# luoao-kddi/SCP

Measured on AMD Instinct MI355X. Metric: KITTI frames/sec encode (SCP-EHEM, level 16) + bpp match vs ref, higher is better.
Workload: dtype f32 (dense layers and attention as bf16x3 split on bf16 MFMA, feature kNN as f16x3 split on f16 MFMA, fp32 accumulate; position kNN / CDF in fp32); 1 GPU; SCP-EHEM KITTI-like synthetic 120k-pt frames, --spher --mullevel lidar_level=16 (BASELINE.json configs[2]), seeded random weights; nodes_per_frame=577403, windows_per_frame=100, frames_per_gpu=46, frames_in_flight=4, frames_per_launch_sequence=1, transform=host-numpy on a prefetch thread (strict identity: the reference's integers), parallelism=frame-sharded x1, rank_cores=256, rank_cores_pinned=False

## Files before the change

include/scp.h:

```cpp
#ifndef SCP_H
#define SCP_H
#include <stddef.h>
#include <stdint.h>

#ifdef __cplusplus
extern "C" {
#endif

#define SCP_API __attribute__((visibility("default")))

#define SCP_OK 0
#define SCP_EINVAL (-1)
#define SCP_ENOMEM (-2)
#define SCP_ESMALL (-3)
#define SCP_EHIP (-4)
#define SCP_ESTATE (-5)

#define SCP_MAX_DEPTH 21
#define SCP_MAX_SEGMENTS 62

#define SCP_ABI_VERSION 220
SCP_API int scp_version(void);
SCP_API int scp_last_hip_error(void);
SCP_API int scp_device_count(void);
// ... 338 lines not shown
    double mn, den;
} scp_expand_seg;
SCP_API int scp_decode_expand_batch(const int64_t *sym, const int64_t *cum, const int32_t *pos, const uint8_t *anc, const uint8_t *octant,
                                    int64_t n, const scp_expand_seg *seg, int32_t S, int32_t cs, const int64_t *wbase, int32_t K, int64_t M,
                                    int64_t T, void *table_dev, int32_t *cpos, uint8_t *canc, uint8_t *coct, uint8_t *cctx, float *cposn,
                                    uint8_t *occ8, void *stream);

SCP_API int scp_swin_ln_linear(const float *x, int64_t ldx, const float *valid, const void *Whi, const void *Wlo, const float *bias,
                               const float *wbeta, float eps, float *out, int64_t ldo, int32_t M, int32_t N, void *stream);
SCP_API int scp_swin_post_attn(const void *Ohi, const void *Olo, int64_t ldo_in, const float *x, int64_t ldx, const void *W, const float *bp,
                               const float *b1, const float *b2, float eps, float *out, int64_t ldc, int32_t M, const int32_t *tile_list,
                               int32_t n_tiles, void *stream);
SCP_API int64_t scp_swin_post_attn_weight_bytes(void);
SCP_API double scp_gelu_prescale(void);

SCP_API int scp_swin_merge(const float *x, int64_t ldx, int64_t n_src, const int64_t *ia, const int64_t *ib, const void *W, const float *wbeta,
                           float eps, float *out, int64_t ldo, int32_t M, void *stream);

SCP_API int scp_geo_edge_mlps(const float *pos1, int64_t ld1, const float *pos2, int64_t ld2, const float *pos3, int64_t ld3, const void *W,
                              const float *bias, float *out, int64_t ldo, int32_t M, void *stream);
SCP_API int scp_mlp3_rows(const float *x, int64_t ldx, int64_t n_src, const int64_t *in_map, const void *W, const float *bias, float *out, int64_t ldo,
                          const int64_t *out_map, int32_t M, int32_t N, void *stream);

SCP_API int scp_swin_kv_planes(const float *k, const float *v, int64_t ldkv, int64_t rows, void *khi, void *klo, void *vthi, void *vtlo, void *stream);
SCP_API int scp_swin_ln_qkv(const float *x, int64_t ldx, const float *valid, const void *Whi, const void *Wlo, const float *bias, const float *wbeta,
                            float eps, float *q, int64_t ldq, void *planes, int64_t Tp, int32_t M, int32_t N, void *stream);
SCP_API int scp_swin_attention_packed_planes(const float *q, const void *khi, const void *klo, const void *vthi, const void *vtlo,
                                             const float *bias_table, const int32_t *wtab, int32_t total_windows, int32_t shift, int32_t ldq,
                                             float *out, void *ohi, void *olo, int64_t ldo, const float *valid, void *stream);

#ifdef __cplusplus
}
#endif
#endif
```

scp_amd/csrc/attn.hip:

```cpp
#include <stdlib.h>
#include "scp_internal.h"

typedef float f32x16 __attribute__((ext_vector_type(16)));

#define WIN 512
#define HD 64
#define NH 4
#define QT 128
#define KT 64
#define LDK 68

typedef __bf16 bf16x4s __attribute__((ext_vector_type(4)));
__device__ __forceinline__ void store_split4(__bf16 *hi, __bf16 *lo, float a, float b, float c, float d) {
    float f[4] = {a, b, c, d};
#pragma unroll
    for (int u = 0; u < 4; ++u) asm volatile("" : "+v"(f[u]));
    bf16x4s vh, vl;
#pragma unroll
    for (int u = 0; u < 4; ++u) {
        const __bf16 hh = (__bf16)f[u];
        vh[u] = hh;
        vl[u] = (__bf16)(f[u] - (float)hh);
    }
    *(bf16x4s *)hi = vh;
// ... 218 lines not shown
#pragma unroll
        for (int j = 0; j < 8; ++j) {
            const float x = f[j] * (0.125f * LOG2E);
            const __bf16 hh = (__bf16)x;
            qh[c][j] = hh;
            ql[c][j] = (__bf16)(x - (float)hh);
        }
    }
}

__device__ __forceinline__ void attn_store_o(const f32x16 &o0, const f32x16 &o1, float inv, int h, float *dst ,
                                             __bf16 *ohi, __bf16 *olo ) {
#pragma unroll
    for (int g = 0; g < 4; ++g) {
        const int d = 8 * g + 4 * h;
        if (ohi) {
            store_split4(ohi + d, olo + d, o0[4 * g] * inv, o0[4 * g + 1] * inv, o0[4 * g + 2] * inv, o0[4 * g + 3] * inv);
            store_split4(ohi + 32 + d, olo + 32 + d, o1[4 * g] * inv, o1[4 * g + 1] * inv, o1[4 * g + 2] * inv, o1[4 * g + 3] * inv);
        } else {
            *(float4 *)(dst + d) = make_float4(o0[4 * g] * inv, o0[4 * g + 1] * inv, o0[4 * g + 2] * inv, o0[4 * g + 3] * inv);
            *(float4 *)(dst + 32 + d) = make_float4(o1[4 * g] * inv, o1[4 * g + 1] * inv, o1[4 * g + 2] * inv, o1[4 * g + 3] * inv);
        }
    }
}

template <bool FASTFIRST>
__global__ __launch_bounds__(256, 2) void swin_attn_bf16x3_kernel(const float *__restrict__ q, const float *__restrict__ k,
                                                                 const float *__restrict__ v, const float *__restrict__ table,
                                                                 int Lp, int shift, int ldq, int ldkv, float *__restrict__ out,
                                                                 const int *__restrict__ wtab, __bf16 *__restrict__ ohi,
                                                                 __bf16 *__restrict__ olo, int64_t ldo) {
    __shared__ __attribute__((aligned(16))) __bf16 Kh[KT * LDB], Kl[KT * LDB];
    __shared__ __attribute__((aligned(16))) __bf16 Vh[HD * LDB], Vl[HD * LDB];
    __shared__ float tab[2 * WIN - 1];

    const int tid = threadIdx.x, w = tid >> 6, lane = tid & 63, col = lane & 31, h = lane >> 5;
    int bid = blockIdx.x;
    bid = (bid & 7) * (int)(gridDim.x >> 3) + (bid >> 3);
    const int qtile = bid & 3; bid >>= 2;
    const int head = bid & 3; bid >>= 2;
    size_t seq_row;
    int wnd, nW;
    if (wtab) { seq_row = (size_t)wtab[2 * bid]; Lp = wtab[2 * bid + 1]; nW = Lp / WIN; wnd = (int)(((size_t)bid * WIN - seq_row) / WIN); }
    else { nW = Lp / WIN; wnd = bid % nW; seq_row = (size_t)(bid / nW) * Lp; }
    const size_t base = seq_row * (NH * HD) + head * HD;
    const size_t qbase = seq_row * ldq + head * HD, kbase = seq_row * ldkv + head * HD;
// ... 149 lines not shown
        for (int t = 0; t < WIN / PKT; ++t) {
            if (PNS > 2 && t + 1 < WIN / PKT) SCP_BARRIER_DMA(4); else SCP_BARRIER_DMA(0);
            if (t + PNS - 1 < WIN / PKT) issue(t + PNS - 1, (t + PNS - 1) % PNS);
            const char *S = stg + (t % PNS) * PST;
            const float madd = (masked && ((t * PKT) >> 8) != qreg) ? -100.f * LOG2E : 0.f;
            auto kfrag = [&](int c, bf16x8 &ah, bf16x8 &al) {
                const int ko = col * 128 + (((2 * c + h) ^ (col & 7)) << 4);
                ah = *(const bf16x8 *)(S + ko); al = *(const bf16x8 *)(S + 4096 + ko);
            };
            auto vfrag = [&](int c, bf16x8 &v0h, bf16x8 &v0l, bf16x8 &v1h, bf16x8 &v1l) {
                const int R0 = col >> 1, R1 = R0 + 16, sl = (col & 1) * 4 + 2 * c + h;
                const int v0 = R0 * 128 + ((sl ^ (R0 & 7)) << 4), v1 = R1 * 128 + ((sl ^ (R1 & 7)) << 4);
                v0h = *(const bf16x8 *)(S + 8192 + v0); v0l = *(const bf16x8 *)(S + 12288 + v0);
                v1h = *(const bf16x8 *)(S + 8192 + v1); v1l = *(const bf16x8 *)(S + 12288 + v1);
            };
            attn_tile<FAST>(kfrag, vfrag, qh, ql, tab, qi - (t * PKT + 4 * h) + (WIN - 1), madd, h, o0, o1, m_run, l_run);
        }
    };
    if (FASTFIRST) {
        sweep(AttnFast{});
        if (__syncthreads_or(!attn_fast_ok(l_run, o0, o1, h))) sweep(AttnStd{});
    } else sweep(AttnStd{});
    const float inv = 1.0f / l_run;
    attn_store_o(o0, o1, inv, h, out ? out + base + (size_t)qtok * (NH * HD) : nullptr,
                 ohi ? ohi + (seq_row + (size_t)qtok) * (size_t)ldo + head * HD : nullptr, ohi ? olo + (seq_row + (size_t)qtok) * (size_t)ldo + head * HD : nullptr);
}

__global__ __launch_bounds__(256) void kv_planes_kernel(const float *__restrict__ k, const float *__restrict__ v, int64_t ldkv, int64_t rows,
                                                       __bf16 *__restrict__ khi, __bf16 *__restrict__ klo, __bf16 *__restrict__ vthi,
                                                       __bf16 *__restrict__ vtlo) {
    const int64_t g = (int64_t)blockIdx.x * 256 + threadIdx.x;
    if (g >= rows * 32) return;
    const int64_t row = g >> 5;
    const int head = (int)(g >> 3) & 3, ch = (int)g & 7;
    const float *ks = k + row * ldkv + head * HD + 8 * ch, *vs = v + row * ldkv + head * HD + 8 * ch;
    const float4 a = *(const float4 *)ks, b = *(const float4 *)(ks + 4), c = *(const float4 *)vs, d = *(const float4 *)(vs + 4);
    const float kf[8] = {a.x, a.y, a.z, a.w, b.x, b.y, b.z, b.w}, vf[8] = {c.x, c.y, c.z, c.w, d.x, d.y, d.z, d.w};
    bf16x8 kh, kl;
#pragma unroll
    for (int u = 0; u < 8; ++u) { const __bf16 hh = (__bf16)kf[u]; kh[u] = hh; kl[u] = (__bf16)(kf[u] - (float)hh); }
    const int64_t ko = row * (NH * HD) + head * HD + ((ch ^ (int)(row & 7)) << 3);
    *(bf16x8 *)(khi + ko) = kh;
    *(bf16x8 *)(klo + ko) = kl;
    const int kk = (int)(row & 31), p = (kk & ~12) | ((kk & 4) << 1) | ((kk & 8) >> 1);
    const int64_t vb = ((row >> 5) * NH + head) * (int64_t)2048;
#pragma unroll
// ... 6 lines not shown
    }
}

extern "C" SCP_API int scp_swin_kv_planes(const float *k, const float *v, int64_t ldkv, int64_t rows, void *khi, void *klo, void *vthi, void *vtlo,
                                          void *stream) {
    if (!k || !v || !khi || !klo || !vthi || !vtlo || rows <= 0 || (rows & 31) || ldkv < NH * HD || (ldkv & 3) ||
        (((uintptr_t)k | (uintptr_t)v | (uintptr_t)khi | (uintptr_t)klo | (uintptr_t)vthi | (uintptr_t)vtlo) & 15))
        return SCP_EINVAL;
    hipLaunchKernelGGL(kv_planes_kernel, dim3((unsigned)cdiv64(rows * 32, 256)), dim3(256), 0, (hipStream_t)stream, k, v, ldkv, rows, (__bf16 *)khi,
                       (__bf16 *)klo, (__bf16 *)vthi, (__bf16 *)vtlo);
    LAUNCH_CHECK();
    return SCP_OK;
}

static std::atomic<int> g_attn_variant{1};
extern "C" SCP_API int scp_set_attention_variant(int32_t v) { g_attn_variant.store(v ? 1 : 0, std::memory_order_relaxed); return SCP_OK; }
extern "C" SCP_API int scp_get_attention_variant(void) { return g_attn_variant.load(std::memory_order_relaxed); }

extern "C" SCP_API int scp_swin_attention_packed_planes(const float *q, const void *khi, const void *klo, const void *vthi, const void *vtlo,
                                                        const float *bias_table, const int32_t *wtab, int32_t total_windows, int32_t shift, int32_t ldq,
                                                        float *out, void *ohi, void *olo, int64_t ldo, const float *valid, void *stream) {
    if (!q || !khi || !klo || !vthi || !vtlo || !bias_table || !wtab || (!out && !ohi) || total_windows <= 0 || (shift != 0 && shift != WIN / 2) ||
        ldq < NH * HD || (ldq & 3) || (((uintptr_t)q | (uintptr_t)out | (uintptr_t)khi | (uintptr_t)klo | (uintptr_t)vthi | (uintptr_t)vtlo) & 15) ||
        (ohi && (!olo || ldo < NH * HD || (ldo & 3) || (((uintptr_t)ohi | (uintptr_t)olo) & 7))))
        return SCP_EINVAL;
    SCP_PROF(SCP_PROF_ATTENTION, stream, (double)total_windows * WIN * 2.0 * 2.0 * WIN * NH * HD);
#define ATTN_GO(V) hipLaunchKernelGGL(swin_attn_planes_kernel<V>, dim3(total_windows * NH * (WIN / QT)), dim3(256), PNS * PST, (hipStream_t)stream, q, (const __bf16 *)khi, \
                                      (const __bf16 *)klo, (const __bf16 *)vthi, (const __bf16 *)vtlo, bias_table, shift, ldq, out, wtab, (__bf16 *)ohi, (__bf16 *)olo, ldo, valid)
    if (g_attn_variant.load(std::memory_order_relaxed) == 0) ATTN_GO(false); else ATTN_GO(true);
#undef ATTN_GO
    LAUNCH_CHECK();
    return SCP_OK;
}

static int g_attn_mode = -1;
static inline bool attn_bf16x3() {
    const int c = scp_ctx_attention_mode();
    if (c >= 0) return c == 1;
    if (g_attn_mode < 0) { const char *e = getenv("SCP_ATTN"); g_attn_mode = (e && e[0] == 'f') ? 0 : 1; }
    return g_attn_mode == 1;
}
extern "C" SCP_API int scp_set_attention_mode(int32_t bf16x3) { g_attn_mode = bf16x3 ? 1 : 0; return SCP_OK; }

static int attn_packed(const float *q, const float *k, const float *v, const float *bias_table, const int32_t *wtab, int32_t total_windows,
                       int32_t shift, int32_t ldq, int32_t ldkv, float *out, __bf16 *ohi, __bf16 *olo, int64_t ldo, void *stream) {
    if (!q || !k || !v || !bias_table || (!out && !ohi) || !wtab || total_windows <= 0 || (shift != 0 && shift != WIN / 2) || ldq < NH * HD ||
        ldkv < NH * HD || (ldq & 3) || (ldkv & 3) || (((uintptr_t)q | (uintptr_t)k | (uintptr_t)v | (uintptr_t)out) & 15) ||
// ... 49 lines not shown
```

scp_amd/csrc/rowchain.hip:

```cpp
#include <stdlib.h>
#include "scp_internal.h"
#include "rc_common.h"

#define RC_SLOT 32768
#define RC_RING (4 * RC_SLOT)
#define RC_OFF_BOUNCE RC_RING
#define RC_OFF_BIAS (RC_RING + 4 * RC_BOUNCE)
#define RC_LDS (RC_OFF_BIAS + 16384)

__device__ __forceinline__ void rc_issue_rowchunk(const RcLane &L, const __bf16 *Whi, const __bf16 *Wlo, int g, char *slot) {
#pragma unroll
    for (int j = 0; j < 4; ++j) {
        const int p = L.w + 4 * j;
        const int64_t off = ((int64_t)g * 16 + p) * 512 + L.lane * 8;
        rc_dma16(Whi + off, slot + p * 1024);
        rc_dma16(Wlo + off, slot + 16384 + p * 1024);
    }
}

__device__ __forceinline__ void rc_issue_kchunk(const RcLane &L, const __bf16 *Whi, const __bf16 *Wlo, int c, int nks, char *slot) {
#pragma unroll
    for (int j = 0; j < 4; ++j) {
        const int p = L.w + 4 * j;
        const int64_t off = ((int64_t)p * nks + c) * 512 + L.lane * 8;
// ... 548 lines not shown
            if (gap == 5) RC_MFMA_AVV(Y[blk], A[s & 1][2], Hch[t]);
            RC_SB;
            if (s < 15 && RC_PROBE_FRAG_ON) {
                if (gap == 0 && HAS_P1) RC_DS_READ(A[nb][1], (ns & 1) ? f.r1 : f.r0, 16384 + (ns >> 1) * 1024);
                if (gap == 1) RC_DS_READ(A[nb][3], (ns & 1) ? f.k1 : f.k0, RC_SLOT + 16384 + (ns >> 1) * 2048);
                if (gap == 2 && HAS_P1) RC_DS_READ(A[nb][0], (ns & 1) ? f.r1 : f.r0, (ns >> 1) * 1024);
                if (gap == 3) RC_DS_READ(A[nb][2], (ns & 1) ? f.k1 : f.k0, RC_SLOT + (ns >> 1) * 2048);
            }
            if (RC_DMA_HERE(s, gap) && RC_PROBE_DMA_ON) rc_dma_piece(L, wr, RC_DMA_SLOT(s, gap) ? n1 : n0, nxt + RC_DMA_SLOT(s, gap) * RC_SLOT, RC_DMA_IDX(s, gap), RC_DMA_PLANE(s, gap));
            if (HAS_GELU) {
                const int k = s >> 1, st = (s & 1) * 6 + gap;
                unsigned wh = 0, wl = 0;
                rc_gelu_stage(st, g, a1g[2 * k], a1g[2 * k + 1], wh, wl);
                if (st == 10) Hnh[k >> 2][k & 3] = wh;
                if (st == 11) Hnl[k >> 2][k & 3] = wl;
            }
            RC_SB;
        }
    }
    if (NEXT == 0) RC_DS_READ4_WAIT(A[0][1], fn.r0, 16384, A[0][3], fn.k0, RC_SLOT + 16384, A[0][0], fn.r0, 0, A[0][2], fn.k0, RC_SLOT);
    else RC_DS_READ4_WAIT(A[0][1], fn.r0, 16384, A[0][3], fn.r0, RC_SLOT + 16384, A[0][0], fn.r0, 0, A[0][2], fn.r0, RC_SLOT);
}

__global__ __launch_bounds__(256, 1) void rc_post_attn_kernel(const RcPostArgs a) {
    extern __shared__ __attribute__((aligned(1024))) char smem[];
    const RcLane L = rc_lane();
    const int ntiles = (a.M + RC_ROWS - 1) / RC_ROWS;
    float *sbp = (float *)(smem + RC_OFF_BIAS), *sb2 = sbp + 256, *sb1 = sbp + 512;
    for (int i = threadIdx.x; i < 256; i += 256) { sbp[i] = a.bp[i]; sb2[i] = a.b2[i]; }
    for (int i = threadIdx.x; i < 1024; i += 256) sb1[i] = a.b1[i];
    __syncthreads();
    const int nlist = a.tile_list ? a.n_list : ntiles;
    auto tile_of = [&](int i) { return a.tile_list ? a.tile_list[i] : i; };
    int ti = blockIdx.x;
    if (ti >= nlist) return;
    int tile = tile_of(ti);
    char *bounce = smem + RC_OFF_BOUNCE + L.w * RC_BOUNCE;
    const int ldc_bytes = (int)(a.ldc * 4);
    const int voff = (32 * L.w + (L.lane >> 3)) * ldc_bytes + (L.lane & 7) * 16;

    const __amdgpu_buffer_rsrc_t wr = __builtin_amdgcn_make_buffer_rsrc((void *)a.W, 0, 2 * RC_W_PLANE, 0x00020000);
    auto src_p = [&](int g) { RcSlotSrc r = {RC_W_PROJ + g * 16384, 1024}; return r; };
    auto src_1 = [&](int c) { RcSlotSrc r = {RC_W_FC1 + c * 16384, 1024}; return r; };
    auto src_2 = [&](int c) { RcSlotSrc r = {RC_W_FC2 + c * 1024, 32 * 1024}; return r; };

    unsigned long long t_p0 = 0, t_ln = 0, t_mlp = 0, t_epi = 0, t_prev = 0, n_tiles = 0;
    const bool DBG = a.dbg != nullptr;
    unsigned long long t_first = 0, r_first = 0;
    if (DBG) { t_prev = t_first = __builtin_amdgcn_s_memtime(); r_first = __builtin_amdgcn_s_memrealtime(); }
    auto stamp = [&](unsigned long long &acc_t) { if (DBG) { const unsigned long long t = __builtin_amdgcn_s_memtime(); acc_t += t - t_prev; t_prev = t; } };

    {
        const RcSlotSrc s0 = src_p(0), s1 = src_p(1);
#pragma unroll
        for (int q = 0; q < 4; ++q)
#pragma unroll
            for (int plane = 0; plane < 2; ++plane) { rc_dma_piece(L, wr, s0, smem, q, plane); rc_dma_piece(L, wr, s1, smem + RC_SLOT, q, plane); }
    }
    rbf16x8 Bh[16], Bl[16];
    auto load_o = [&](int t) {
        const int r0 = t * RC_ROWS + 32 * L.w + (L.lane >> 3);
#pragma unroll
        for (int it = 0; it < 4; ++it) {
            const int r = r0 + 8 * it;
            const int64_t o = (int64_t)(r < a.M ? r : a.M - 1) * a.ldo_in + (L.lane & 7) * 8;
#pragma unroll
            for (int pp = 0; pp < 4; ++pp) { Bh[4 * pp + it] = *(const rbf16x8 *)(a.Ohi + o + 64 * pp); Bl[4 * pp + it] = *(const rbf16x8 *)(a.Olo + o + 64 * pp); }
        }
    };
    auto transpose_o = [&]() {
#pragma unroll
        for (int plane = 0; plane < 2; ++plane)
#pragma unroll
            for (int pp = 0; pp < 4; ++pp) {
#pragma unroll
                for (int it = 0; it < 4; ++it) {
                    const int rho = 8 * it + (L.lane >> 3), kap = L.lane & 7;
                    *(rbf16x8 *)(bounce + rho * 128 + ((kap ^ (rho & 7)) << 4)) = plane ? Bl[4 * pp + it] : Bh[4 * pp + it];
                }
                asm volatile("s_waitcnt lgkmcnt(0)" ::: "memory");
#pragma unroll
                for (int q = 0; q < 4; ++q) {
                    const rbf16x8 fr = *(const rbf16x8 *)(bounce + L.col * 128 + (((2 * q + L.h) ^ (L.col & 7)) << 4));
                    if (plane) Bl[4 * pp + q] = fr; else Bh[4 * pp + q] = fr;
                }
                asm volatile("s_waitcnt lgkmcnt(0)" ::: "memory");
            }
    };
    load_o(tile);
    transpose_o();
    rbf16x8 A[2][4];
    {
        SCP_BARRIER_DMA(0);
// ... 156 lines not shown
#pragma unroll
                for (int u = 0; u < 4; ++u) o[q][u] = Y[b][4 * q + u];
            rc_store_block(L, bounce, o, rs, ldc_bytes, voff, 32 * b);
        }
        transpose_o();
        stamp(t_epi);
        ++n_tiles;
    }
    if (DBG && L.lane == 0) {
        unsigned long long *o = a.dbg + ((size_t)blockIdx.x * 4 + L.w) * 8;
        o[0] = t_p0; o[1] = t_mlp; o[2] = t_ln; o[3] = t_epi; o[4] = n_tiles;
        o[5] = __builtin_amdgcn_s_memtime() - t_first; o[6] = __builtin_amdgcn_s_memrealtime() - r_first;
    }
    SCP_WAIT_DMA(0);
}

#ifndef RCW_D1
#define RCW_D1 4
#endif
#ifndef RCW_D2
#define RCW_D2 2
#endif
#define RCW_H_BYTES (32 * 4096)
__global__ __launch_bounds__(256, 1) void rc_post_attn_wide_kernel(const RcPostArgs a) {
    extern __shared__ __attribute__((aligned(1024))) char smem[];
    const RcLane L = rc_lane();
    float *sbp = (float *)(smem + RC_OFF_BIAS), *sb2 = sbp + 256, *sb1 = sbp + 512;
    for (int i = threadIdx.x; i < 256; i += 256) { sbp[i] = a.bp[i]; sb2[i] = a.b2[i]; }
    for (int i = threadIdx.x; i < 1024; i += 256) sb1[i] = a.b1[i];
    __syncthreads();
    const int n128 = a.tile_list ? a.n_list : (a.M + RC_ROWS - 1) / RC_ROWS;
    char *bounce = smem + RC_OFF_BOUNCE + L.w * RC_BOUNCE;
    char *hbuf = smem;
    const int ldc_bytes = (int)(a.ldc * 4);
    const int voff = (L.lane >> 3) * ldc_bytes + (L.lane & 7) * 16;
    const __amdgpu_buffer_rsrc_t wr = __builtin_amdgcn_make_buffer_rsrc((void *)a.W, 0, 2 * RC_W_PLANE, 0x00020000);
    const int vrc0 = L.rg * 8192 + L.frag, vrc1 = L.rg * 8192 + (L.frag ^ 32);
    const int vkc0 = L.rg * 32768 + L.frag, vkc1 = L.rg * 32768 + (L.frag ^ 32);
    auto wload = [&](int voff, int soff) { return __builtin_bit_cast(rbf16x8, __builtin_amdgcn_raw_buffer_load_b128(wr, voff, soff, 0)); };
    for (int item = blockIdx.x; item < 4 * n128; item += gridDim.x) {
        const int t128 = a.tile_list ? a.tile_list[item >> 2] : (item >> 2);
        const int m0 = t128 * RC_ROWS + 32 * (item & 3);
        if (m0 >= a.M) continue;
        rbf16x8 Bh[16], Bl[16];
        {
            const int r0 = m0 + (L.lane >> 3);
#pragma unroll
            for (int it = 0; it < 4; ++it) {
                const int r = r0 + 8 * it;
                const int64_t o = (int64_t)(r < a.M ? r : a.M - 1) * a.ldo_in + (L.lane & 7) * 8;
#pragma unroll
                for (int pp = 0; pp < 4; ++pp) { Bh[4 * pp + it] = *(const rbf16x8 *)(a.Ohi + o + 64 * pp); Bl[4 * pp + it] = *(const rbf16x8 *)(a.Olo + o + 64 * pp); }
            }
#pragma unroll
            for (int plane = 0; plane < 2; ++plane)
#pragma unroll
                for (int pp = 0; pp < 4; ++pp) {
#pragma unroll
                    for (int it = 0; it < 4; ++it) {
                        const int rho = 8 * it + (L.lane >> 3), kap = L.lane & 7;
                        *(rbf16x8 *)(bounce + rho * 128 + ((kap ^ (rho & 7)) << 4)) = plane ? Bl[4 * pp + it] : Bh[4 * pp + it];
                    }
                    asm volatile("s_waitcnt lgkmcnt(0)" ::: "memory");
#pragma unroll
                    for (int q = 0; q < 4; ++q) {
                        const rbf16x8 fr = *(const rbf16x8 *)(bounce + L.col * 128 + (((2 * q + L.h) ^ (L.col & 7)) << 4));
                        if (plane) Bl[4 * pp + q] = fr; else Bh[4 * pp + q] = fr;
                    }
// ... 629 lines not shown
        (q && (int64_t)RC_ROWS * ldq * 4 > 0x7fffffffLL) || 4 * Tp * 512 > 0x7fffffffLL)
        return SCP_EINVAL;
    static bool configured = false;
    if (!configured) {
        HIP_TRY(hipFuncSetAttribute((const void *)rc_ln_linear_kernel<0, true>, hipFuncAttributeMaxDynamicSharedMemorySize, RC_LDS));
        configured = true;
    }
    RcLnLinArgs a;
    a.x = x; a.ldx = ldx; a.valid = valid; a.Whi = (const __bf16 *)Whi; a.Wlo = (const __bf16 *)Wlo; a.bias = bias; a.wbeta = wbeta;
    a.out = q; a.ldo = q ? ldq : 256; a.M = M; a.N = N; a.eps = eps; a.probe = 0; a.dbg = nullptr;
    a.planes = (__bf16 *)planes; a.plane_bytes = Tp * 512; a.nq = N / 64 - 8;
    const int ntiles = M / RC_ROWS, ncu = rc_num_cu();
    SCP_PROF(SCP_PROF_LN_LINEAR, stream, 2.0 * M * 256.0 * N);
    if (rc_lnlin2_here(ntiles, ncu)) return scp_lnlin2_launch(a, true, ncu, (hipStream_t)stream);
    a.ngroups = rc_ll_groups(ntiles, N / 64, ncu);
    hipLaunchKernelGGL((rc_ln_linear_kernel<0, true>), dim3((unsigned)(a.ngroups > 1 ? ntiles * a.ngroups : (ntiles < ncu ? ntiles : ncu))), dim3(256), RC_LDS, (hipStream_t)stream, a);
    LAUNCH_CHECK();
    return SCP_OK;
}

extern "C" SCP_API int scp_swin_post_attn(const void *Ohi, const void *Olo, int64_t ldo_in, const float *x, int64_t ldx, const void *W, const float *bp,
                                          const float *b1, const float *b2, float eps, float *out, int64_t ldc, int32_t M, const int32_t *tile_list,
                                          int32_t n_tiles, void *stream) {
    if (!Ohi || !Olo || !x || !W || !bp || !b1 || !b2 || !out || M <= 0 || (tile_list && (n_tiles <= 0 || n_tiles > (M + RC_ROWS - 1) / RC_ROWS)) || ldo_in < 256 || (ldo_in & 7) || ldx < 256 || (ldx & 3) || ldc < 256 ||
        (ldc & 3) || (((uintptr_t)Ohi | (uintptr_t)Olo | (uintptr_t)x | (uintptr_t)out | (uintptr_t)W) & 15) ||
        (int64_t)RC_ROWS * ldc * 4 > 0x7fffffffLL)
        return SCP_EINVAL;
    static bool configured = false;
    if (!configured) {
        HIP_TRY(hipFuncSetAttribute((const void *)rc_post_attn_kernel, hipFuncAttributeMaxDynamicSharedMemorySize, RC_LDS));
        HIP_TRY(hipFuncSetAttribute((const void *)rc_post_attn_wide_kernel, hipFuncAttributeMaxDynamicSharedMemorySize, RC_LDS));
        configured = true;
    }
    RcPostArgs a;
    a.Ohi = (const __bf16 *)Ohi; a.Olo = (const __bf16 *)Olo; a.ldo_in = ldo_in; a.x = x; a.ldx = ldx; a.W = W;
    a.bp = bp; a.b1 = b1; a.b2 = b2; a.out = out; a.ldc = ldc; a.M = M; a.eps = eps;
    a.dbg = g_rc_dbg;
    { const char *e = getenv("SCP_RC_DUMP"); a.dbg_mode = e ? atoi(e) : 0; }
    a.tile_list = tile_list; a.n_list = tile_list ? n_tiles : 0;
    const int ntiles = tile_list ? n_tiles : (M + RC_ROWS - 1) / RC_ROWS;
    const int ncu = rc_num_cu();
    SCP_PROF(SCP_PROF_POST_ATTN, stream, 2.0 * (tile_list ? (double)n_tiles * RC_ROWS : (double)M) * (256.0 * 256.0 + 2.0 * 256.0 * 1024.0));
    if (rc_wide_mode() == 1 || (rc_wide_mode() < 0 && !g_rc_dbg && !a.dbg_mode && 4 * (int64_t)ntiles <= (int64_t)ncu)) {
        const int items = 4 * ntiles;
        hipLaunchKernelGGL(rc_post_attn_wide_kernel, dim3((unsigned)(items < 2 * ncu ? items : 2 * ncu)), dim3(256), RC_LDS, (hipStream_t)stream, a);
        LAUNCH_CHECK();
        return SCP_OK;
    }
    hipLaunchKernelGGL(rc_post_attn_kernel, dim3((unsigned)(ntiles < ncu ? ntiles : ncu)), dim3(256), RC_LDS, (hipStream_t)stream, a);
    LAUNCH_CHECK();
    return SCP_OK;
}

extern "C" SCP_API int64_t scp_swin_post_attn_weight_bytes(void) { return 2 * (int64_t)RC_W_PLANE; }

extern "C" SCP_API int scp_geo_edge_mlps(const float *pos1, int64_t ld1, const float *pos2, int64_t ld2, const float *pos3, int64_t ld3, const void *W,
                                         const float *bias, float *out, int64_t ldo, int32_t M, void *stream) {
    if (!pos1 || !pos2 || !pos3 || !W || !bias || !out || M <= 0 || ld1 < 64 || ld2 < 128 || ld3 < 256 || ((ld1 | ld2 | ld3) & 3) || ldo < 128 || (ldo & 3) ||
        (((uintptr_t)pos1 | (uintptr_t)pos2 | (uintptr_t)pos3 | (uintptr_t)out | (uintptr_t)W) & 15) || (int64_t)RC_ROWS * ldo * 4 > 0x7fffffffLL)
        return SCP_EINVAL;
    static bool configured = false;
    if (!configured) {
        HIP_TRY(hipFuncSetAttribute((const void *)rc_edge_mlp_kernel, hipFuncAttributeMaxDynamicSharedMemorySize, RC_LDS));
        configured = true;
    }
    RcEdgeArgs a;
    a.p1 = pos1; a.p2 = pos2; a.p3 = pos3; a.ld1 = ld1; a.ld2 = ld2; a.ld3 = ld3; a.W = W; a.bias = bias; a.out = out; a.ldo = ldo; a.M = M;
    const int ntiles = (M + RC_ROWS - 1) / RC_ROWS, ncu = rc_num_cu();
    SCP_PROF(SCP_PROF_EDGE_MLP, stream, 2.0 * M * (448.0 * 256 + 2.0 * 256 * 256 + 512.0 * 256 + 256.0 * 256 + 256.0 * 128));
    hipLaunchKernelGGL(rc_edge_mlp_kernel, dim3((unsigned)(ntiles < ncu ? ntiles : ncu)), dim3(256), RC_LDS, (hipStream_t)stream, a);
    LAUNCH_CHECK();
    return SCP_OK;
// ... 40 lines not shown
```

scp_amd/models/packed.py:

```python
import numpy as np
import torch
import torch.nn.functional as F

from .. import native
from ..ops import linear_s, leaky_mlp3_s, split_cat, linear, layer_norm, leaky_mlp3, _split, derived, frozen_epoch
from .ehem import SHIFT, WINDOW, _edge_conv_packed, qkv_fused


def _ceil512(a):
    return (a + WINDOW - 1) // WINDOW * WINDOW


def _tokens(L):
    wid = torch.repeat_interleave(torch.arange(L.numel(), device=L.device), L)
    first = torch.cumsum(L, 0) - L
    return wid, torch.arange(int(L.sum()), device=L.device) - first[wid]


class StageLayout:

    def __init__(self, L):
        self.L = L
        self.Lp = _ceil512(L)
        self.base = torch.cumsum(self.Lp, 0) - self.Lp
# ... 106 lines not shown
def _block_consts(layer, cross):
    ep = frozen_epoch()
    key = "_scp_fast_x" if cross else "_scp_fast"
    fast = layer.__dict__.get(key) if ep else None
    if fast is not None and fast[0] == ep:
        return fast[1:]
    att = layer.attention.self
    out = (_rowchain_weights(layer, cross), att.relative_position_bias_table, (att.query.bias if cross else None), layer.layernorm_before.eps, layer.layernorm_after.eps)
    if ep:
        layer.__dict__[key] = (ep,) + out
    return out


def _swin_layer_rowchain(layer, x, valid, wtab, shift, query=None, tiles=None, q_pre=None):
    cross = query is not None
    w, table, qbias, eps_b, eps_a = _block_consts(layer, cross)
    v1 = None if valid is None else valid.reshape(-1)
    if native.attention_bf16x3():
        if not cross:
            q, kvp = native.swin_ln_qkv(x, w["kv"], w["b"], eps_b, v1)
        else:
            q = q_pre if q_pre is not None else native.swin_ln_linear(query, w["q"], qbias, eps_b, v1)
            _, kvp = native.swin_ln_qkv(x, w["kv"], w["b"], eps_b, v1)
        o = native.swin_attention_packed_planes(q, kvp, table, wtab, shift, split=True, valid=v1 if tiles is not None else None)
        if tiles is not None and tiles.shape[0] > 0:
            return native.swin_post_attn(o, x, w["post"], eps_a, out=x, tiles=tiles)
        return native.swin_post_attn(o, x, w["post"], eps_a)
    att, lnb = layer.attention.self, layer.layernorm_before
    if not cross:
        qkv = native.swin_ln_linear(x, w["kv"], w["b"], lnb.eps, v1)
        q, k, v = qkv[:, :256], qkv[:, 256:512], qkv[:, 512:]
    else:
        q = q_pre if q_pre is not None else native.swin_ln_linear(query, w["q"], att.query.bias, lnb.eps, v1)
        kv = native.swin_ln_linear(x, w["kv"], w["b"], lnb.eps, v1)
        k, v = kv[:, :256], kv[:, 256:]
    o = native.swin_attention_packed(q, k, v, att.relative_position_bias_table, wtab, shift, split=True)
    return native.swin_post_attn(o, x, w["post"], layer.layernorm_after.eps)


def _swin_layer(layer, x, valid, wtab, shift, query=None, tiles=None, q_pre=None):
    fc1, fc2 = layer.intermediate.dense, layer.output.dense
    if x.shape[1] != 256 or fc1.weight.shape != (1024, 256) or fc2.weight.shape != (256, 1024):
        raise native.ScpError("EHEM's Swin blocks are 256 wide with a 1024-wide MLP (configs/model/ehem.yaml); other widths are not built")
    return _swin_layer_rowchain(layer, x, valid, wtab, shift, query, tiles, q_pre)


def _merge(m, x, maps):
# ... 213 lines not shown
```

scp_amd/native.py:

```python
import ctypes as C
import os

import numpy as np
import torch

HERE = os.path.dirname(os.path.abspath(__file__))
LIB_PATH = os.path.join(HERE, "libscp_hip.so")
MAX_DEPTH = 21

CART, SPHER, CYLIN = 0, 1, 2
POS_MINMAX, POS_MINMAX_MUL, POS_POW2 = 0, 1, 2
_ERR = {-1: "SCP_EINVAL", -2: "SCP_ENOMEM", -3: "SCP_ESMALL", -4: "SCP_EHIP", -5: "SCP_ESTATE"}


class ScpError(RuntimeError):
    pass


class QuantInfo(C.Structure):
    _fields_ = [("bin_num", C.c_double), ("qs", C.c_double * 3), ("offset", C.c_double * 3),
                ("max_coord", C.c_int32), ("min_coord", C.c_int32)]


class Segment(C.Structure):
# ... 396 lines not shown
                                                   o.t[1].data_ptr(), o.t.stride(1), _stream())
        _check(rc, "scp_swin_attention_packed_split")
        return o
    out = torch.empty((T, 256), dtype=torch.float32, device=q.device)
    rc = lib().scp_swin_attention_packed(q.data_ptr(), k.data_ptr(), v.data_ptr(), _dev(bias_table, torch.float32),
                                         _dev(wtab, torch.int32), T // 512, shift, q.stride(0), k.stride(0), _dev(out), _stream())
    _check(rc, "scp_swin_attention_packed")
    return out


class KvPlanes:

    __slots__ = ("t",)

    def __init__(self, k=None, v=None, t=None):
        if t is None:
            T = k.shape[0]
            t = torch.empty((4, T, 256), dtype=torch.bfloat16, device=k.device)
            _check(lib().scp_swin_kv_planes(k.data_ptr(), v.data_ptr(), k.stride(0), T, t[0].data_ptr(), t[1].data_ptr(), t[2].data_ptr(),
                                            t[3].data_ptr(), _stream()), "scp_swin_kv_planes")
        self.t = t


def swin_attention_packed_planes(q, kv, bias_table, wtab, shift, split=False, valid=None):
    T = q.shape[0]
    p = kv.t
    vp = None if valid is None else _dev(valid, torch.float32)
    if split:
        o = SplitAct.empty(T, 256, q.device)
        rc = lib().scp_swin_attention_packed_planes(q.data_ptr(), p[0].data_ptr(), p[1].data_ptr(), p[2].data_ptr(), p[3].data_ptr(),
                                                    _dev(bias_table, torch.float32), _dev(wtab, torch.int32), T // 512, shift, q.stride(0), None,
                                                    o.t[0].data_ptr(), o.t[1].data_ptr(), o.t.stride(1), vp, _stream())
        _check(rc, "scp_swin_attention_packed_planes")
        return o
    out = torch.empty((T, 256), dtype=torch.float32, device=q.device)
    rc = lib().scp_swin_attention_packed_planes(q.data_ptr(), p[0].data_ptr(), p[1].data_ptr(), p[2].data_ptr(), p[3].data_ptr(),
                                                _dev(bias_table, torch.float32), _dev(wtab, torch.int32), T // 512, shift, q.stride(0), _dev(out), None,
                                                None, 0, vp, _stream())
    _check(rc, "scp_swin_attention_packed_planes")
    return out


def nn_sqdist(a, b):
    a = _dev_f64(a)
    b = _dev_f64(b)
    out = torch.empty((a.shape[0],), dtype=torch.float64, device=a.device)
    _check(lib().scp_nn_sqdist_f64(a.data_ptr(), a.shape[0], b.data_ptr(), b.shape[0], out.data_ptr(), _stream()), "scp_nn_sqdist_f64")
    return out


# ... 757 lines not shown
        perm_k, perm_h = rc_perm16(256, dev), rc_perm16(w1.shape[0], dev)
        w1d = w1.detach().double()
        s = float(lib().scp_gelu_prescale())
        swp = SplitWeight(wp.detach().float().contiguous())
        sw1 = SplitWeight((w1d * gamma.detach().double()[None, :] * s).float()[:, perm_k].contiguous())
        sw2 = SplitWeight((w2.detach().double() / s).float()[:, perm_h].contiguous())
        tiles = [_tiled_planes_always(w) for w in (swp, sw1, sw2)]
        self.packed = torch.cat([t[0].reshape(-1) for t in tiles] + [t[1].reshape(-1) for t in tiles]).contiguous()
        if self.packed.numel() * 2 != lib().scp_swin_post_attn_weight_bytes():
            raise ScpError("swin_post_attn: 256 -> 1024 -> 256 blocks only")
        self.bp = bp.detach().float().contiguous()
        self.b1 = ((b1.detach().double() + w1d @ beta.detach().double()) * s).float().contiguous()
        self.b2 = b2.detach().float().contiguous()
        note_cache_fill()


def swin_post_attn(o, x, pw, eps=1e-5, out=None, tiles=None):
    M = x.shape[0]
    if o.K != 256 or o.M != M or x.shape[1] != 256 or x.stride(1) != 1:
        raise ScpError("swin_post_attn: [M, 256] operands expected")
    if out is None:
        out = torch.empty((M, 256), dtype=torch.float32, device=x.device)
    t = o.t
    rc = lib().scp_swin_post_attn(t[0].data_ptr(), t[1].data_ptr(), t.stride(1), x.data_ptr(), x.stride(0), pw.packed.data_ptr(), _dev(pw.bp),
                                  _dev(pw.b1), _dev(pw.b2), float(eps), out.data_ptr(), out.stride(0), M,
                                  None if tiles is None else _dev(tiles, torch.int32), 0 if tiles is None else int(tiles.shape[0]), _stream())
    _check(rc, "scp_swin_post_attn")
    return out


def layernorm_rows(x, gamma, beta, eps=1e-5, valid=None, ia=None, ib=None, out=None, split=False):
    Cc = gamma.shape[0]
    rows = x.shape[0] if ia is None else ia.shape[0]
    if split:
        o = SplitAct.empty(rows, Cc, x.device)
        rc = lib().scp_layernorm_rows_split(x.data_ptr(), x.stride(0), x.shape[0], None if ia is None else _dev(ia, torch.int64),
                                            None if ib is None else _dev(ib, torch.int64), Cc, _dev(gamma), _dev(beta),
                                            None if valid is None else _dev(valid, torch.float32), float(eps), o.t[0].data_ptr(),
                                            o.t[1].data_ptr(), o.t.stride(1), rows, _stream())
        _check(rc, "scp_layernorm_rows_split")
        return o
    if out is None:
        out = torch.empty((rows, Cc), dtype=torch.float32, device=x.device)
    rc = lib().scp_layernorm_rows(x.data_ptr(), x.stride(0), x.shape[0], None if ia is None else _dev(ia, torch.int64),
                                  None if ib is None else _dev(ib, torch.int64), Cc, _dev(gamma), _dev(beta),
                                  None if valid is None else _dev(valid, torch.float32), float(eps), out.data_ptr(), out.stride(0),
                                  rows, _stream())
# ... 911 lines not shown
```

Baseline: 15.98 frames/s.

## Hand attention output to post-attn kernel in MFMA fragment layout

Adds a fragment-ordered layout for the bf16 hi/lo attention output. The attention kernel writes it with permlane32 swaps, and the post-attention kernel loads it straight into MFMA B registers through buffer loads. This removes the LDS transpose and the strided row loads in the post-attention kernels, at the cost of a new tiled tensor format and extra API mode plumbing (ldo==0 sentinel). It is on by default, and the old row layout stays available through an environment variable.

```diff
diff --git a/include/scp.h b/include/scp.h
--- a/include/scp.h
+++ b/include/scp.h
@@ -384,6 +384,7 @@
 SCP_API int scp_mlp3_rows(const float *x, int64_t ldx, int64_t n_src, const int64_t *in_map, const void *W, const float *bias, float *out, int64_t ldo,
                           const int64_t *out_map, int32_t M, int32_t N, void *stream);
 
+#define SCP_LDO_FRAG 0
 SCP_API int scp_swin_kv_planes(const float *k, const float *v, int64_t ldkv, int64_t rows, void *khi, void *klo, void *vthi, void *vtlo, void *stream);
 SCP_API int scp_swin_ln_qkv(const float *x, int64_t ldx, const float *valid, const void *Whi, const void *Wlo, const float *bias, const float *wbeta,
                             float eps, float *q, int64_t ldq, void *planes, int64_t Tp, int32_t M, int32_t N, void *stream);
diff --git a/scp_amd/csrc/attn.hip b/scp_amd/csrc/attn.hip
--- a/scp_amd/csrc/attn.hip
+++ b/scp_amd/csrc/attn.hip
@@ -264,6 +264,39 @@
             *(float4 *)(dst + 32 + d) = make_float4(o1[4 * g] * inv, o1[4 * g + 1] * inv, o1[4 * g + 2] * inv, o1[4 * g + 3] * inv);
         }
     }
+}
+
+__device__ __forceinline__ void attn_store_o_frag(const f32x16 &o0, const f32x16 &o1, float inv, __bf16 *ohi, __bf16 *olo) {
+    typedef unsigned attn_u32x4 __attribute__((ext_vector_type(4)));
+    typedef unsigned attn_u32x2 __attribute__((ext_vector_type(2)));
+#pragma unroll
+    for (int half = 0; half < 2; ++half)
+#pragma unroll
+        for (int gp = 0; gp < 2; ++gp) {
+            attn_u32x2 ph[2], pl[2];
+#pragma unroll
+            for (int e = 0; e < 2; ++e) {
+                float f[4];
+#pragma unroll
+                for (int u = 0; u < 4; ++u) f[u] = (half ? o1[8 * gp + 4 * e + u] : o0[8 * gp + 4 * e + u]) * inv;
+#pragma unroll
+                for (int u = 0; u < 4; ++u) asm volatile("" : "+v"(f[u]));
+                bf16x4s vh, vl;
+#pragma unroll
+                for (int u = 0; u < 4; ++u) {
+                    const __bf16 hh = (__bf16)f[u];
+                    vh[u] = hh;
+                    vl[u] = (__bf16)(f[u] - (float)hh);
+                }
+                ph[e] = __builtin_bit_cast(attn_u32x2, vh);
+                pl[e] = __builtin_bit_cast(attn_u32x2, vl);
+            }
+            const auto h0 = __builtin_amdgcn_permlane32_swap(ph[0][0], ph[1][0], false, false), h1 = __builtin_amdgcn_permlane32_swap(ph[0][1], ph[1][1], false, false);
+            const auto l0 = __builtin_amdgcn_permlane32_swap(pl[0][0], pl[1][0], false, false), l1 = __builtin_amdgcn_permlane32_swap(pl[0][1], pl[1][1], false, false);
+            const int64_t c = (int64_t)(4 * half + 2 * gp) * 1024;
+            *(attn_u32x4 *)(ohi + c) = (attn_u32x4){h0[0], h1[0], h0[1], h1[1]};
+            *(attn_u32x4 *)(olo + c) = (attn_u32x4){l0[0], l1[0], l0[1], l1[1]};
+        }
 }
 
 template <bool FASTFIRST>
@@ -459,6 +492,12 @@
         if (__syncthreads_or(!attn_fast_ok(l_run, o0, o1, h))) sweep(AttnStd{});
     } else sweep(AttnStd{});
     const float inv = 1.0f / l_run;
+    if (ohi && ldo == 0) {
+        const size_t row = seq_row + (size_t)qtok;
+        const size_t e = (((row >> 7) * 32 + head * 8 + h) * 128 + (row & 127)) * 8;
+        attn_store_o_frag(o0, o1, inv, ohi + e, olo + e);
+        return;
+    }
     attn_store_o(o0, o1, inv, h, out ? out + base + (size_t)qtok * (NH * HD) : nullptr,
                  ohi ? ohi + (seq_row + (size_t)qtok) * (size_t)ldo + head * HD : nullptr, ohi ? olo + (seq_row + (size_t)qtok) * (size_t)ldo + head * HD : nullptr);
 }
@@ -511,7 +550,8 @@
                                                         float *out, void *ohi, void *olo, int64_t ldo, const float *valid, void *stream) {
     if (!q || !khi || !klo || !vthi || !vtlo || !bias_table || !wtab || (!out && !ohi) || total_windows <= 0 || (shift != 0 && shift != WIN / 2) ||
         ldq < NH * HD || (ldq & 3) || (((uintptr_t)q | (uintptr_t)out | (uintptr_t)khi | (uintptr_t)klo | (uintptr_t)vthi | (uintptr_t)vtlo) & 15) ||
-        (ohi && (!olo || ldo < NH * HD || (ldo & 3) || (((uintptr_t)ohi | (uintptr_t)olo) & 7))))
+        (ohi && ldo != SCP_LDO_FRAG && (!olo || ldo < NH * HD || (ldo & 3) || (((uintptr_t)ohi | (uintptr_t)olo) & 7))) ||
+        (ohi && ldo == SCP_LDO_FRAG && (!olo || (((uintptr_t)ohi | (uintptr_t)olo) & 15))))
         return SCP_EINVAL;
     SCP_PROF(SCP_PROF_ATTENTION, stream, (double)total_windows * WIN * 2.0 * 2.0 * WIN * NH * HD);
 #define ATTN_GO(V) hipLaunchKernelGGL(swin_attn_planes_kernel<V>, dim3(total_windows * NH * (WIN / QT)), dim3(256), PNS * PST, (hipStream_t)stream, q, (const __bf16 *)khi, \
diff --git a/scp_amd/csrc/rowchain.hip b/scp_amd/csrc/rowchain.hip
--- a/scp_amd/csrc/rowchain.hip
+++ b/scp_amd/csrc/rowchain.hip
@@ -594,6 +594,17 @@
     else RC_DS_READ4_WAIT(A[0][1], fn.r0, 16384, A[0][3], fn.r0, RC_SLOT + 16384, A[0][0], fn.r0, 0, A[0][2], fn.r0, RC_SLOT);
 }
 
+__device__ __forceinline__ void rc_load_o_frag(const __bf16 *Ohi, const __bf16 *Olo, int tile, int r, int h, rbf16x8 (&Bh)[16], rbf16x8 (&Bl)[16]) {
+    const __amdgpu_buffer_rsrc_t rh = __builtin_amdgcn_make_buffer_rsrc((void *)(Ohi + (int64_t)tile * (RC_ROWS * 256)), 0, RC_ROWS * 512, 0x00020000);
+    const __amdgpu_buffer_rsrc_t rl = __builtin_amdgcn_make_buffer_rsrc((void *)(Olo + (int64_t)tile * (RC_ROWS * 256)), 0, RC_ROWS * 512, 0x00020000);
+    const int v = (r & (RC_ROWS - 1)) * 16 + h * 2048;
+#pragma unroll
+    for (int s = 0; s < 16; ++s) Bh[s] = __builtin_bit_cast(rbf16x8, __builtin_amdgcn_raw_buffer_load_b128(rh, v, 4096 * s, 0));
+#pragma unroll
+    for (int s = 0; s < 16; ++s) Bl[s] = __builtin_bit_cast(rbf16x8, __builtin_amdgcn_raw_buffer_load_b128(rl, v, 4096 * s, 0));
+}
+
+template <bool OFRAG>
 __global__ __launch_bounds__(256, 1) void rc_post_attn_kernel(const RcPostArgs a) {
     extern __shared__ __attribute__((aligned(1024))) char smem[];
     const RcLane L = rc_lane();
@@ -631,6 +642,11 @@
     }
     rbf16x8 Bh[16], Bl[16];
     auto load_o = [&](int t) {
+        if (OFRAG) {
+            const int r = t * RC_ROWS + 32 * L.w + L.col;
+            rc_load_o_frag(a.Ohi, a.Olo, t, r < a.M ? r : a.M - 1, L.h, Bh, Bl);
+            return;
+        }
         const int r0 = t * RC_ROWS + 32 * L.w + (L.lane >> 3);
 #pragma unroll
         for (int it = 0; it < 4; ++it) {
@@ -641,6 +657,11 @@
         }
     };
     auto transpose_o = [&]() {
+        if (OFRAG) {
+#pragma unroll
+            for (int s = 0; s < 16; ++s) asm volatile("" : "+v"(Bh[s]), "+v"(Bl[s]));
+            return;
+        }
 #pragma unroll
         for (int plane = 0; plane < 2; ++plane)
 #pragma unroll
@@ -843,6 +864,7 @@
 #define RCW_D2 2
 #endif
 #define RCW_H_BYTES (32 * 4096)
+template <bool OFRAG>
 __global__ __launch_bounds__(256, 1) void rc_post_attn_wide_kernel(const RcPostArgs a) {
     extern __shared__ __attribute__((aligned(1024))) char smem[];
     const RcLane L = rc_lane();
@@ -864,7 +886,10 @@
         const int m0 = t128 * RC_ROWS + 32 * (item & 3);
         if (m0 >= a.M) continue;
         rbf16x8 Bh[16], Bl[16];
-        {
+        if (OFRAG) {
+            const int r = m0 + L.col;
+            rc_load_o_frag(a.Ohi, a.Olo, t128, r < a.M ? r : a.M - 1, L.h, Bh, Bl);
+        } else {
             const int r0 = m0 + (L.lane >> 3);
 #pragma unroll
             for (int it = 0; it < 4; ++it) {
@@ -1540,14 +1565,16 @@
 extern "C" SCP_API int scp_swin_post_attn(const void *Ohi, const void *Olo, int64_t ldo_in, const float *x, int64_t ldx, const void *W, const float *bp,
                                           const float *b1, const float *b2, float eps, float *out, int64_t ldc, int32_t M, const int32_t *tile_list,
                                           int32_t n_tiles, void *stream) {
-    if (!Ohi || !Olo || !x || !W || !bp || !b1 || !b2 || !out || M <= 0 || (tile_list && (n_tiles <= 0 || n_tiles > (M + RC_ROWS - 1) / RC_ROWS)) || ldo_in < 256 || (ldo_in & 7) || ldx < 256 || (ldx & 3) || ldc < 256 ||
+    if (!Ohi || !Olo || !x || !W || !bp || !b1 || !b2 || !out || M <= 0 || (tile_list && (n_tiles <= 0 || n_tiles > (M + RC_ROWS - 1) / RC_ROWS)) || (ldo_in != SCP_LDO_FRAG && (ldo_in < 256 || (ldo_in & 7))) || ldx < 256 || (ldx & 3) || ldc < 256 ||
         (ldc & 3) || (((uintptr_t)Ohi | (uintptr_t)Olo | (uintptr_t)x | (uintptr_t)out | (uintptr_t)W) & 15) ||
         (int64_t)RC_ROWS * ldc * 4 > 0x7fffffffLL)
         return SCP_EINVAL;
     static bool configured = false;
     if (!configured) {
-        HIP_TRY(hipFuncSetAttribute((const void *)rc_post_attn_kernel, hipFuncAttributeMaxDynamicSharedMemorySize, RC_LDS));
-        HIP_TRY(hipFuncSetAttribute((const void *)rc_post_attn_wide_kernel, hipFuncAttributeMaxDynamicSharedMemorySize, RC_LDS));
+        HIP_TRY(hipFuncSetAttribute((const void *)rc_post_attn_kernel<true>, hipFuncAttributeMaxDynamicSharedMemorySize, RC_LDS));
+        HIP_TRY(hipFuncSetAttribute((const void *)rc_post_attn_kernel<false>, hipFuncAttributeMaxDynamicSharedMemorySize, RC_LDS));
+        HIP_TRY(hipFuncSetAttribute((const void *)rc_post_attn_wide_kernel<true>, hipFuncAttributeMaxDynamicSharedMemorySize, RC_LDS));
+        HIP_TRY(hipFuncSetAttribute((const void *)rc_post_attn_wide_kernel<false>, hipFuncAttributeMaxDynamicSharedMemorySize, RC_LDS));
         configured = true;
     }
     RcPostArgs a;
@@ -1556,16 +1583,19 @@
     a.dbg = g_rc_dbg;
     { const char *e = getenv("SCP_RC_DUMP"); a.dbg_mode = e ? atoi(e) : 0; }
     a.tile_list = tile_list; a.n_list = tile_list ? n_tiles : 0;
+    const bool frag = ldo_in == SCP_LDO_FRAG;
     const int ntiles = tile_list ? n_tiles : (M + RC_ROWS - 1) / RC_ROWS;
     const int ncu = rc_num_cu();
     SCP_PROF(SCP_PROF_POST_ATTN, stream, 2.0 * (tile_list ? (double)n_tiles * RC_ROWS : (double)M) * (256.0 * 256.0 + 2.0 * 256.0 * 1024.0));
     if (rc_wide_mode() == 1 || (rc_wide_mode() < 0 && !g_rc_dbg && !a.dbg_mode && 4 * (int64_t)ntiles <= (int64_t)ncu)) {
         const int items = 4 * ntiles;
-        hipLaunchKernelGGL(rc_post_attn_wide_kernel, dim3((unsigned)(items < 2 * ncu ? items : 2 * ncu)), dim3(256), RC_LDS, (hipStream_t)stream, a);
+        if (frag) hipLaunchKernelGGL(rc_post_attn_wide_kernel<true>, dim3((unsigned)(items < 2 * ncu ? items : 2 * ncu)), dim3(256), RC_LDS, (hipStream_t)stream, a);
+        else hipLaunchKernelGGL(rc_post_attn_wide_kernel<false>, dim3((unsigned)(items < 2 * ncu ? items : 2 * ncu)), dim3(256), RC_LDS, (hipStream_t)stream, a);
         LAUNCH_CHECK();
         return SCP_OK;
     }
-    hipLaunchKernelGGL(rc_post_attn_kernel, dim3((unsigned)(ntiles < ncu ? ntiles : ncu)), dim3(256), RC_LDS, (hipStream_t)stream, a);
+    if (frag) hipLaunchKernelGGL(rc_post_attn_kernel<true>, dim3((unsigned)(ntiles < ncu ? ntiles : ncu)), dim3(256), RC_LDS, (hipStream_t)stream, a);
+    else hipLaunchKernelGGL(rc_post_attn_kernel<false>, dim3((unsigned)(ntiles < ncu ? ntiles : ncu)), dim3(256), RC_LDS, (hipStream_t)stream, a);
     LAUNCH_CHECK();
     return SCP_OK;
 }
diff --git a/scp_amd/models/packed.py b/scp_amd/models/packed.py
--- a/scp_amd/models/packed.py
+++ b/scp_amd/models/packed.py
@@ -152,7 +152,7 @@
         else:
             q = q_pre if q_pre is not None else native.swin_ln_linear(query, w["q"], qbias, eps_b, v1)
             _, kvp = native.swin_ln_qkv(x, w["kv"], w["b"], eps_b, v1)
-        o = native.swin_attention_packed_planes(q, kvp, table, wtab, shift, split=True, valid=v1 if tiles is not None else None)
+        o = native.swin_attention_packed_planes(q, kvp, table, wtab, shift, split=native.attn_o_split(), valid=v1 if tiles is not None else None)
         if tiles is not None and tiles.shape[0] > 0:
             return native.swin_post_attn(o, x, w["post"], eps_a, out=x, tiles=tiles)
         return native.swin_post_attn(o, x, w["post"], eps_a)
diff --git a/scp_amd/native.py b/scp_amd/native.py
--- a/scp_amd/native.py
+++ b/scp_amd/native.py
@@ -442,10 +442,62 @@
         self.t = t
 
 
+_ATTN_O = "rows" if os.environ.get("SCP_ATTN_O", "")[:1] == "r" else "frag"
+LDO_FRAG = 0
+
+
+def set_attn_o(mode):
+    global _ATTN_O
+    if mode not in ("frag", "rows"):
+        raise ScpError("attention output hand-over: 'frag' or 'rows'")
+    prev, _ATTN_O = _ATTN_O, mode
+    return prev
+
+
+def attn_o_split():
+    return "frag" if _ATTN_O == "frag" else True
+
+
+class FragAct:
+
+    __slots__ = ("t", "M", "K")
+
+    def __init__(self, t, M):
+        self.t, self.M, self.K = t, M, 256
+
+    @staticmethod
+    def empty(M, device):
+        return FragAct(torch.empty((2, -(-M // 128), 32, 128, 8), dtype=torch.bfloat16, device=device), M)
+
+    @staticmethod
+    def from_rows(a):
+        M = a.M
+        nt = -(-M // 128)
+        r = torch.zeros((2, nt * 128, 256), dtype=torch.bfloat16, device=a.t.device)
+        r[:, :M] = a.t[:, :, :256]
+        return FragAct(r.view(2, nt, 128, 32, 8).permute(0, 1, 3, 2, 4).contiguous(), M)
+
+    def rows(self):
+        nt = self.t.shape[1]
+        return SplitAct(self.t.permute(0, 1, 3, 2, 4).reshape(2, nt * 128, 256)[:, :self.M].contiguous(), 256)
+
+    def float(self):
+        return self.rows().float()
+
+
 def swin_attention_packed_planes(q, kv, bias_table, wtab, shift, split=False, valid=None):
     T = q.shape[0]
     p = kv.t
     vp = None if valid is None else _dev(valid, torch.float32)
+    if isinstance(split, str):
+        if split != "frag":
+            raise ScpError("swin_attention_packed_planes: split is False, True or 'frag'")
+        o = FragAct.empty(T, q.device)
+        rc = lib().scp_swin_attention_packed_planes(q.data_ptr(), p[0].data_ptr(), p[1].data_ptr(), p[2].data_ptr(), p[3].data_ptr(),
+                                                    _dev(bias_table, torch.float32), _dev(wtab, torch.int32), T // 512, shift, q.stride(0), None,
+                                                    o.t[0].data_ptr(), o.t[1].data_ptr(), LDO_FRAG, vp, _stream())
+        _check(rc, "scp_swin_attention_packed_planes")
+        return o
     if split:
         o = SplitAct.empty(T, 256, q.device)
         rc = lib().scp_swin_attention_packed_planes(q.data_ptr(), p[0].data_ptr(), p[1].data_ptr(), p[2].data_ptr(), p[3].data_ptr(),
@@ -1249,7 +1301,8 @@
     if out is None:
         out = torch.empty((M, 256), dtype=torch.float32, device=x.device)
     t = o.t
-    rc = lib().scp_swin_post_attn(t[0].data_ptr(), t[1].data_ptr(), t.stride(1), x.data_ptr(), x.stride(0), pw.packed.data_ptr(), _dev(pw.bp),
+    ldo = LDO_FRAG if isinstance(o, FragAct) else t.stride(1)
+    rc = lib().scp_swin_post_attn(t[0].data_ptr(), t[1].data_ptr(), ldo, x.data_ptr(), x.stride(0), pw.packed.data_ptr(), _dev(pw.bp),
                                   _dev(pw.b1), _dev(pw.b2), float(eps), out.data_ptr(), out.stride(0), M,
                                   None if tiles is None else _dev(tiles, torch.int32), 0 if tiles is None else int(tiles.shape[0]), _stream())
     _check(rc, "scp_swin_post_attn")
```

Result: faster. 16.37 frames/s, median of 6 (+2.4%).
